# Fil/nd4js

Hardware: AMD Instinct MI355X
Metric: fp64 GFLOP/s: matmul N=4096 & SVD N=2048; % of MFMA/HBM peak (higher is better)
Workload: dtype f64; 1 GPU; matmul 4096x4096x4096 fp64, one matrix pair per GPU (BASELINE configs[1]); parallelism=batch-sharded x1, no collective, inputs=uniform(-1,1) seeds 5/6, HBM-resident

## Files before the change

nd4js_amd/csrc/svd.hip:

```cpp
#include "svd_internal.h"
#include "dpp.h"
#include <cmath>
#include <cfloat>
#include <cstring>

namespace {

constexpr int MAX_SWEEPS = 60;

__device__ __forceinline__ double wave_sum(double v) {
#pragma unroll
  for (int off = 32; off > 0; off >>= 1) v += __shfl_xor(v, off);
  return v;
}

__global__ __launch_bounds__(256) void jac_floor(const double* __restrict__ svr, int N, double tol2, double* __restrict__ floor2) {
  const double* s = svr + (long)blockIdx.x * N;
  double mx = 0.0;
  for (int i = threadIdx.x; i < N; i += 256) mx = fmax(mx, s[i]);
#pragma unroll
  for (int off = 32; off > 0; off >>= 1) mx = fmax(mx, __shfl_xor(mx, off));
  __shared__ double s_mx[4];
  if ((threadIdx.x & 63) == 0) s_mx[threadIdx.x >> 6] = mx;
  __syncthreads();
// ... 209 lines not shown
    __syncthreads();
    const unsigned r = s_rot;
    __syncthreads();
    if (t == 0) s_rot = 0;
    rotations += r;
    converged = r == 0;
    __syncthreads();
  }
  for (int e = t; e < N * N; e += 256) {
    const int r = e / N, c = e % N;
    W[e] = s_w[r * LD + c];
    Ut[e] = s_u[r * LD + c];
  }
  if (t == 0) {
    atomicMax(sweeps_max, (unsigned)sweeps);
    if (!converged) atomicAdd(not_converged, 1u);
    atomicMax(offmax, s_off);
    atomicAdd(rot_total, rotations);
  }
}

int jacobi_square(nd4hip_handle* h, int batch, int N, double* W, double* U, double* sv, double* V,
                  int* sweeps_out, double* offnorm_out) {
  Nd4WsScope scope(h);
  const long sM = (long)N * N;
  void* p = nullptr;
  const bool small = N > 1 && N <= 64;
  const bool blocked = N > 64;
  const int Np = blocked ? ((N + 63) / 64) * 64 : N;
  const bool padded = Np != N;
  const long sMp = (long)Np * Np;
  const size_t nblock = blocked ? nd4_jacobi_block_scratch_doubles(batch, Np) : 0;
  const size_t npad = padded ? (size_t)batch * (2 * sMp + Np) : 0;
  const size_t nd = (size_t)batch * (2 * sM + 2 * N + 1) + nblock + npad;
  const size_t nrank = ((size_t)batch * N + 1) & ~size_t(1);
  ND4_TRY(nd4_ws_alloc(h, nd * sizeof(double) + nrank * sizeof(int) + (size_t)batch * sizeof(JacState) + 96, &p));
  double* Ut = static_cast<double*>(p);
  double* Utp = Ut + (size_t)batch * sM;
  double* svr = Utp + (size_t)batch * sM;
  double* scratch = svr + (size_t)batch * N;
  double* floor2 = scratch + (size_t)batch * N;
  double* bscratch = floor2 + batch;
  double* Wp = bscratch + nblock;
  double* Utpad = Wp + (padded ? (size_t)batch * sMp : 0);
  double* svrp = Utpad + (padded ? (size_t)batch * sMp : 0);
  int* rank = reinterpret_cast<int*>(bscratch + nblock + npad);
  JacState* st = reinterpret_cast<JacState*>(rank + nrank);
  unsigned* active = reinterpret_cast<unsigned*>(st + batch);
  unsigned long long* offmax = reinterpret_cast<unsigned long long*>(active + 2);
  unsigned long long* rot_total = offmax + 1;
  void* pin = nullptr;
  ND4_TRY(nd4_pinned(h, 64 + sizeof(int) * (size_t)batch, &pin));
  unsigned* h_active = static_cast<unsigned*>(pin);
  unsigned long long* h_off = reinterpret_cast<unsigned long long*>(h_active + 2);

  if (!small) ND4_TRY(nd4_set_identity(h, N, N, Ut, N, batch, sM));
  ND4_HIP(hipMemsetAsync(st, 0, sizeof(JacState) * batch + 32, h->stream));
  if (padded) {
    ND4_HIP(hipMemsetAsync(Wp, 0, sizeof(double) * (size_t)batch * sMp, h->stream));
    ND4_TRY(nd4_copy_matrix(h, N, N, W, N, Wp, Np, batch, sM, sMp));
    ND4_TRY(nd4_set_identity(h, Np, Np, Utpad, Np, batch, sMp));
  }
  double* Wb = padded ? Wp : W;
  double* Utb = padded ? Utpad : Ut;

  const double eps = 0x1p-52, tol = N * eps, tol2 = tol * tol;
  if (!small) {
    hipLaunchKernelGGL(jac_norms, dim3((unsigned)((N + 3) / 4), (unsigned)batch), dim3(256), 0, h->stream, W, N, sM, svr);
    hipLaunchKernelGGL(jac_floor, dim3((unsigned)batch), dim3(256), 0, h->stream, svr, N, tol2, floor2);
  }
  int sweeps = 0;
  unsigned long long last_off = 0, rot_seen = 0;
  bool dense_phase = blocked && Np >= 512;
  if (small) {
    ND4_HIP(hipMemsetAsync(active, 0, 16, h->stream));
// ... 189 lines not shown
```

nd4js_amd/csrc/svd_block.hip:

```cpp
#include "svd_internal.h"
#include <cstdlib>

typedef double d4 __attribute__((ext_vector_type(4)));
typedef double d2 __attribute__((ext_vector_type(2)));

namespace {

constexpr int BB = 32;
constexpr int PB = 64;
constexpr int CH = 256;

template <int K> __device__ __forceinline__ int bcast_i(int v) { return __builtin_amdgcn_readlane(v, K); }
template <int K> __device__ __forceinline__ double bcast_d(double v) {
  return __hiloint2double(__builtin_amdgcn_readlane(__double2hiint(v), K), __builtin_amdgcn_readlane(__double2loint(v), K));
}

__device__ __forceinline__ double fast_rcp(double x) {
  double r = __builtin_amdgcn_rcp(x);
  r = fma(fma(-x, r, 1.0), r, r);
  r = fma(fma(-x, r, 1.0), r, r);
  return r;
}
__device__ __forceinline__ double fast_rsqrt(double x) {
  double r = __builtin_amdgcn_rsq(x);
  r = r * fma(-0.5 * x * r, r, 1.5);
  r = r * fma(-0.5 * x * r, r, 1.5);
  return r;
}

__device__ __forceinline__ long pair_row(int x, int I, int J) { return x < BB ? (long)I * BB + x : (long)J * BB + (x - BB); }

__host__ __device__ __forceinline__ void jacb_pair(int n2, int s, int i, int& I, int& J) {
  if (n2 > 0) { nd4_rr_pair(n2, s, i, I, J); return; }
  const int n = -n2, h = n / 2, q = n / 4;
  const int grp = i >= q ? 1 : 0, ii = i - grp * q;
  if (s < h - 1) {
    nd4_rr_pair(h, s, ii, I, J);
    I += grp * h; J += grp * h;
  } else {
    const int c = s - (h - 1), second = c >= q ? 1 : 0, cc = c - second * q;
    I = grp * q + ii;
    J = h + ((grp ^ second) ? q : 0) + (ii + cc) % q;
  }
}
__host__ __device__ __forceinline__ int jacb_abs(int n2) { return n2 < 0 ? -n2 : n2; }

__device__ __forceinline__ void gram_load_group(d2 (&dst)[2][4], const double* const (&rp)[4], int c) {
#pragma unroll
  for (int t = 0; t < 4; t++) {
    dst[0][t] = *reinterpret_cast<const d2*>(rp[t] + c);
    dst[1][t] = *reinterpret_cast<const d2*>(rp[t] + c + 2);
  }
}
__device__ __forceinline__ void gram_mfma_group(d4 (&acc)[4][4], const d2 (&f)[2][4]) {
#pragma unroll
  for (int u = 0; u < 2; u++)
#pragma unroll
    for (int i = 0; i < 4; i++)
#pragma unroll
      for (int j = i; j < 4; j++) {
        acc[i][j] = __builtin_amdgcn_mfma_f64_16x16x4f64(f[u][i].x, f[u][j].x, acc[i][j], 0, 0, 0);
        acc[i][j] = __builtin_amdgcn_mfma_f64_16x16x4f64(f[u][i].y, f[u][j].y, acc[i][j], 0, 0, 0);
      }
}
__device__ __forceinline__ void gram_accumulate(d4 (&acc)[4][4], const double* const (&rp)[4], int col0, int ncols, int N, int fk) {
  for (int c0 = col0; c0 < col0 + ncols && c0 < N; c0 += 16) {
    d2 f[2][4];
    gram_load_group(f, rp, c0 + 4 * fk);
    gram_mfma_group(acc, f);
  }
}
template <int LDG>
__device__ __forceinline__ void gram_reduce_lds(double (*G)[LDG], const d4 (&acc)[4][4], int wave, int fk, int fx) {
#pragma unroll
  for (int w = 0; w < 4; w++) {
    if (wave == w) {
#pragma unroll
      for (int i = 0; i < 4; i++)
#pragma unroll
        for (int j = i; j < 4; j++)
#pragma unroll
          for (int r = 0; r < 4; r++) {
            const int row = i * 16 + fk + 4 * r, col = j * 16 + fx;
            double* d = &G[row][col];
            const double v = (w == 0) ? acc[i][j][r] : *d + acc[i][j][r];
            *d = v;
            if (w == 3 && j > i) G[col][row] = v;
          }
    }
    __syncthreads();
  }
}

template <int NT>
__device__ __forceinline__ void gram2_tiles(d4 (&acc)[3], const double (*st)[PB + 2], const int (&ti)[3], const int (&tj)[3], int fx, int fk) {
#pragma unroll
  for (int ks = 0; ks < 16; ks++) {
    double f[4];
#pragma unroll
    for (int q = 0; q < 4; q++) f[q] = st[q * 16 + fx][ks * 4 + fk];
#pragma unroll
    for (int n = 0; n < NT; n++) acc[n] = __builtin_amdgcn_mfma_f64_16x16x4f64(f[ti[n]], f[tj[n]], acc[n], 0, 0, 0);
  }
}
__global__ __launch_bounds__(256) void jacb_gram2(const double* __restrict__ Wm, int N, long sM, int nblk, int nblk2, int step,
                                                   const JacState* __restrict__ st, double* __restrict__ Gpart, int nchunks, long sG_mat, int pair0) {
  __shared__ double s_x[2][PB][PB + 2];
  const int pairIdx = blockIdx.x + pair0, chunk = blockIdx.y, mat = blockIdx.z;
  if (st[mat].done) return;
  int I, J;
  jacb_pair(nblk2, step, pairIdx, I, J);
  if (J >= nblk) return;
  const double* W = Wm + mat * sM;
  const int t = threadIdx.x, lane = t & 63, wave = __builtin_amdgcn_readfirstlane(t >> 6);
  const int fx = lane & 15, fk = lane >> 4;
  const double* src[8];
#pragma unroll
  for (int k = 0; k < 8; k++) src[k] = W + pair_row((t >> 5) + 8 * k, I, J) * N + chunk * CH + 2 * (t & 31);
  const int nsub = (N - chunk * CH >= CH) ? CH / 64 : (N - chunk * CH) / 64;
  d2 v[8];
  auto load = [&](int sub) {
#pragma unroll
    for (int k = 0; k < 8; k++) v[k] = *reinterpret_cast<const d2*>(src[k] + sub * 64);
  };
  auto stash = [&](int buf) {
#pragma unroll
    for (int k = 0; k < 8; k++) *reinterpret_cast<d2*>(&s_x[buf][(t >> 5) + 8 * k][2 * (t & 31)]) = v[k];
  };
  d4 acc[3] = {d4{0.0, 0.0, 0.0, 0.0}, d4{0.0, 0.0, 0.0, 0.0}, d4{0.0, 0.0, 0.0, 0.0}};
  if (nsub > 0) { load(0); stash(0); }
  __syncthreads();
  for (int sub = 0; sub < nsub; sub++) {
    if (sub + 1 < nsub) load(sub + 1);
    const double (*sx)[PB + 2] = s_x[sub & 1];
    if (wave == 0)      { const int ti[3] = {0, 0, 0}, tj[3] = {0, 1, 2}; gram2_tiles<3>(acc, sx, ti, tj, fx, fk); }
    else if (wave == 1) { const int ti[3] = {0, 1, 1}, tj[3] = {3, 1, 2}; gram2_tiles<3>(acc, sx, ti, tj, fx, fk); }
    else if (wave == 2) { const int ti[3] = {1, 2, 2}, tj[3] = {3, 2, 2}; gram2_tiles<2>(acc, sx, ti, tj, fx, fk); }
    else                { const int ti[3] = {2, 3, 3}, tj[3] = {3, 3, 3}; gram2_tiles<2>(acc, sx, ti, tj, fx, fk); }
    if (sub + 1 < nsub) stash((sub + 1) & 1);
    __syncthreads();
  }
  const int TI[4][3] = {{0, 0, 0}, {0, 1, 1}, {1, 2, 2}, {2, 3, 3}};
  const int TJ[4][3] = {{0, 1, 2}, {3, 1, 2}, {3, 2, 2}, {3, 3, 3}};
  double* G = Gpart + mat * sG_mat + ((long)pairIdx * nchunks + chunk) * (PB * PB);
  const int ntiles = wave < 2 ? 3 : 2;
#pragma unroll
  for (int n = 0; n < 3; n++) {
    if (n < ntiles) {
      const int i = TI[wave][n], j = TJ[wave][n];
#pragma unroll
      for (int r = 0; r < 4; r++) G[(i * 16 + fk + 4 * r) * PB + j * 16 + fx] = acc[n][r];
    }
  }
}

template <bool FUSED, int PW>
__global__ __launch_bounds__(2048 / PW) void jacb_eigen(const double* __restrict__ Gpart, int nchunks, long sG_mat, int nblk, int nblk2, int step,
                                                   JacState* __restrict__ st, const double* __restrict__ floor2, double tol2,
                                                   double* __restrict__ Qt_all, long sQ_mat, int* __restrict__ flags, long sF_mat,
                                                   unsigned long long* __restrict__ offmax, int max_inner, int cross_only) {
  __shared__ double G[PB][PB + 1];
  __shared__ double Q[PB][PB + 1];
  __shared__ unsigned s_rot[32 / PW];
  const int pairIdx = blockIdx.x, mat = blockIdx.y;
  if (st[mat].done) return;
  int I, J;
  jacb_pair(nblk2, step, pairIdx, I, J);
  if (J >= nblk) return;
  const int t = threadIdx.x, lane = t & 63, wave = t >> 6;
  if constexpr (FUSED) {
    static_assert(!FUSED || PW == 8, "the fused Gram phase is written for 4 waves");
    const int N = nchunks, fx = lane & 15, fk = lane >> 4;
    const double* W = Gpart + mat * sG_mat;
    const double* rp[4];
#pragma unroll
    for (int q = 0; q < 4; q++) rp[q] = W + pair_row(q * 16 + fx, I, J) * N;
    d4 acc[4][4];
#pragma unroll
    for (int i = 0; i < 4; i++)
#pragma unroll
      for (int j = 0; j < 4; j++) acc[i][j] = d4{0.0, 0.0, 0.0, 0.0};
    const int per = ((N + 63) / 64) * 16;
    gram_accumulate(acc, rp, wave * per, per, N, fk);
    gram_reduce_lds<PB + 1>(G, acc, wave, fk, fx);
    for (int e = t; e < PB * PB; e += 2048 / PW) Q[e / PB][e % PB] = (e / PB == e % PB) ? 1.0 : 0.0;
  } else {
    const double* Gp = Gpart + mat * sG_mat + (long)pairIdx * nchunks * (PB * PB);
    for (int e = t; e < PB * PB; e += 2048 / PW) {
      const int r = e / PB, c = e % PB;
      Q[r][c] = (r == c) ? 1.0 : 0.0;
      if ((r >> 4) > (c >> 4)) continue;
      double s = 0.0;
      for (int ch = 0; ch < nchunks; ch++) s += Gp[(long)ch * (PB * PB) + e];
      G[r][c] = s;
      if ((r >> 4) != (c >> 4)) G[c][r] = s;
    }
  }
  __syncthreads();
  const double fl = floor2[mat];
  unsigned total = 0;
  double relmax = 0.0;
  {
    int need = 0;
    for (int e = t; e < PB * PB; e += 2048 / PW) {
      const int i = e / PB, j = e % PB;
      if (i < j) { const double a = G[i][i], b = G[j][j], g = G[i][j]; need |= (a > fl) && (b > fl) && (g * g > tol2 * a * b); }
    }
    need = __syncthreads_or(need);
    if (!need) { if (t == 0) flags[mat * sF_mat + pairIdx] = 0; return; }
  }
  const int nrounds = cross_only ? BB : PB - 1;
  for (int inner = 0; inner < max_inner; inner++) {
    unsigned rot = 0;
    for (int r = 0; r < nrounds; r++) {
      int p, q;
      if (cross_only) { p = wave * PW + (lane & (PW - 1)); q = BB + ((p + r) & (BB - 1)); }
      else nd4_rr_pair(PB, r, wave * PW + (lane & (PW - 1)), p, q);
      const double a = G[p][p], b = G[q][q], g = G[p][q];
      const bool go = (a > fl) && (b > fl) && (g * g > tol2 * a * b);
      double c = 1.0, s = 0.0;
      if (go) {
        const double d = b - a, hh = 2.0 * g, rr = d * d + hh * hh;
        const double root = rr * fast_rsqrt(rr);
        const double tn = (((d < 0.0) != (g < 0.0)) ? -fabs(hh) : fabs(hh)) * fast_rcp(fabs(d) + root);
        const double cc = fast_rsqrt(1.0 + tn * tn);
        s = cc * tn;
// ... 43 lines not shown
  double* Qt = Qt_all + mat * sQ_mat + (long)pairIdx * (PB * PB);
  if (total) for (int e = t; e < PB * PB; e += 2048 / PW) Qt[e] = Q[e / PB][e % PB];
#pragma unroll
  for (int off = 32; off > 0; off >>= 1) relmax = fmax(relmax, __shfl_xor(relmax, off));
  if (lane == 0 && relmax > 0.0) atomicMax(offmax, (unsigned long long)__double_as_longlong(relmax));
  if (t == 0) {
    flags[mat * sF_mat + pairIdx] = total ? 1 : 0;
    if (total) atomicAdd(&st[mat].rotations, total);
  }
}

template <int CG>
__device__ __forceinline__ void eigen_p_body(double* __restrict__ stage_raw, const int pairIdx, const int mat,
                                             const double* __restrict__ Gpart, int nchunks, long sG_mat, int nblk, int nblk2, int step,
                                             JacState* __restrict__ st, const double* __restrict__ floor2, double tol2,
                                             double* __restrict__ Qt_all, long sQ_mat, int* __restrict__ flags, long sF_mat,
                                             unsigned long long* __restrict__ offmax, int precheck) {
  constexpr int T = 576, TB = 512, NB = 2, NQ = 4;
  constexpr int LD = BB + 1;
  __shared__ double sC[2][BB][LD];
  __shared__ double sB[2][BB][LD];
  __shared__ double sA1[2][BB];
  __shared__ double sAng[2][2][BB];
  double (*stage)[PB + 1] = reinterpret_cast<double (*)[PB + 1]>(stage_raw);
  __shared__ double sRd[PB];
  __shared__ unsigned sTotal;
  double (*QJ)[PB + 1] = stage;
  if (st[mat].done) return;
  int I, J;
  jacb_pair(nblk2, step, pairIdx, I, J);
  if (J >= nblk) return;
  const int t = threadIdx.x, lane = t & 63, wave = t >> 6;
  if (t < TB) {
    constexpr int KL = (PB * PB / 2) / TB;
    const d2* Gp = reinterpret_cast<const d2*>(Gpart + mat * sG_mat + (long)pairIdx * nchunks * (PB * PB));
    d2 acc[KL];
#pragma unroll
    for (int k = 0; k < KL; k++) acc[k] = d2{0.0, 0.0};
    for (int ch0 = 0; ch0 < nchunks; ch0 += CG) {
      d2 v[CG][KL];
#pragma unroll
      for (int c = 0; c < CG; c++)
#pragma unroll
        for (int k = 0; k < KL; k++) {
          const int e = 2 * (t + TB * k);
          v[c][k] = (ch0 + c < nchunks && ((e / PB) >> 4) <= ((e % PB) >> 4)) ? Gp[(long)(ch0 + c) * (PB * PB / 2) + t + TB * k] : d2{0.0, 0.0};
        }
#pragma unroll
      for (int c = 0; c < CG; c++)
#pragma unroll
        for (int k = 0; k < KL; k++) acc[k] += v[c][k];
    }
#pragma unroll
    for (int k = 0; k < KL; k++) {
      const int e = 2 * (t + TB * k), r = e / PB, c = e % PB;
      if ((r >> 4) <= (c >> 4)) {
        stage[r][c] = acc[k].x;
        stage[r][c + 1] = acc[k].y;
        if ((r >> 4) != (c >> 4)) { stage[c][r] = acc[k].x; stage[c + 1][r] = acc[k].y; }
      }
    }
  }
  __syncthreads();
  const double fl = floor2[mat];
  if (precheck) {
    if (t < PB) { const double dd = stage[t][t]; sRd[t] = dd > fl ? __builtin_amdgcn_rcp(dd) : 0.0; }
    __syncthreads();
    double rel = 0.0;
    for (int e = t; e < PB * PB; e += T) {
      const int x = e / PB, y = e % PB;
      const double g = stage[x][y];
      if (x < y) rel = fmax(rel, g * g * sRd[x] * sRd[y]);
    }
#pragma unroll
    for (int off = 32; off > 0; off >>= 1) rel = fmax(rel, __shfl_xor(rel, off));
    if (lane == 0 && rel > 0.0) atomicMax(offmax, (unsigned long long)__double_as_longlong(rel));
    const int need = __syncthreads_or(rel > tol2 * (1.0 - 0x1p-20));
    if (!need) { if (t == 0) flags[mat * sF_mat + pairIdx] = 0; return; }
  }
  const int i = lane & 31, h = lane >> 5;
  const bool pivot = wave == 8;
  const int jb = NB * (2 * wave + h);
  const int cb = NQ * (2 * wave + h);
  double Areg[NB] = {0.0, 0.0}, Qp[NQ] = {0.0, 0.0, 0.0, 0.0};
  double pa = 0.0, pb = 0.0, pg = 0.0;
  if (pivot) {
    pa = stage[i][i]; pb = stage[BB + i][BB + i]; pg = stage[i][BB + i];
  } else {
#pragma unroll
    for (int m = 0; m < NB; m++) Areg[m] = stage[i][jb + m];
#pragma unroll
    for (int m = 0; m < NQ; m++) Qp[m] = (cb + m == i) ? 1.0 : 0.0;
// ... 81 lines not shown
  if (t == 8 * 64) sTotal = rot;
  __syncthreads();
  const unsigned total = sTotal;
  if (total) {
    double* Qt = Qt_all + mat * sQ_mat + (long)pairIdx * (PB * PB);
    if (!pivot) {
#pragma unroll
      for (int m = 0; m < NQ; m++) Qt[i * PB + cb + m] = Qp[m];
    }
    for (int e = t; e < BB * PB; e += T) Qt[BB * PB + e] = QJ[e / PB][e % PB];
  }
  if (t == 0) {
    flags[mat * sF_mat + pairIdx] = total ? 1 : 0;
    if (total) atomicAdd(&st[mat].rotations, total);
  }
}

constexpr int SQ_LD = PB + 4;
constexpr int STAGE_DOUBLES = PB * SQ_LD;
template <int T, int STRIPS = 4>
__device__ __forceinline__ void apply_body(double* __restrict__ sq_raw, const int pairIdx, int chunk, const int mat,
                                           double* __restrict__ Wm, double* __restrict__ Utm, int N, long sM, int nblk, int nblk2, int step,
                                           const JacState* __restrict__ st, const double* __restrict__ Qt_all, long sQ_mat,
                                           const int* __restrict__ flags, long sF_mat, int nchunks) {
  double (*sQ)[SQ_LD] = reinterpret_cast<double (*)[SQ_LD]>(sq_raw);
  if (st[mat].done || !flags[mat * sF_mat + pairIdx]) return;
  int I, J;
  jacb_pair(nblk2, step, pairIdx, I, J);
  if (J >= nblk) return;
  double* X = (chunk < nchunks ? Wm : Utm) + mat * sM;
  if (chunk >= nchunks) chunk -= nchunks;
  const int t = threadIdx.x, lane = t & 63, wave = t >> 6;
  const int fx = lane & 15, fk = lane >> 4;
  const double* Qt = Qt_all + mat * sQ_mat + (long)pairIdx * (PB * PB);
  for (int e = t; e < PB * PB; e += T) sQ[e / PB][e % PB] = Qt[e];
  __syncthreads();
  if (T > 256 && t >= 256) return;
  long rowoff[16];
#pragma unroll
  for (int ks = 0; ks < 16; ks++) rowoff[ks] = pair_row(ks * 4 + fk, I, J) * N;
  const int colw = chunk * (64 * STRIPS) + wave * (16 * STRIPS);
  for (int strip = 0; strip < STRIPS; strip++) {
    const int cbase = colw + strip * 16;
    if (cbase >= N) break;
    const int c = cbase + fx;
    double b[16];
#pragma unroll
    for (int ks = 0; ks < 16; ks++) b[ks] = X[rowoff[ks] + c];
#pragma unroll
    for (int it = 0; it < 4; it++) {
      d4 acc = d4{0.0, 0.0, 0.0, 0.0};
#pragma unroll
      for (int ks = 0; ks < 16; ks++)
        acc = __builtin_amdgcn_mfma_f64_16x16x4f64(sQ[it * 16 + fx][ks * 4 + fk], b[ks], acc, 0, 0, 0);
#pragma unroll
      for (int r = 0; r < 4; r++) X[pair_row(it * 16 + fk + 4 * r, I, J) * N + c] = acc[r];
    }
  }
}

__global__ __launch_bounds__(576) void jacb_eigen_p(const double* __restrict__ Gpart, int nchunks, long sG_mat, int nblk, int nblk2, int step,
                                                     JacState* __restrict__ st, const double* __restrict__ floor2, double tol2,
                                                     double* __restrict__ Qt_all, long sQ_mat, int* __restrict__ flags, long sF_mat,
                                                     unsigned long long* __restrict__ offmax, int precheck, int pair0) {
  __shared__ double stage_raw[STAGE_DOUBLES];
  eigen_p_body<4>(stage_raw, blockIdx.x + pair0, blockIdx.y, Gpart, nchunks, sG_mat, nblk, nblk2, step, st, floor2, tol2, Qt_all, sQ_mat, flags, sF_mat,
               offmax, precheck);
}

__global__ __launch_bounds__(256) void jacb_apply(double* __restrict__ Wm, double* __restrict__ Utm, int N, long sM, int nblk, int nblk2, int step,
                                                   const JacState* __restrict__ st, const double* __restrict__ Qt_all, long sQ_mat,
                                                   const int* __restrict__ flags, long sF_mat, int nchunks, int chunk0, int pair0) {
  __shared__ double sq_raw[STAGE_DOUBLES];
  apply_body<256>(sq_raw, blockIdx.x + pair0, blockIdx.y + chunk0, blockIdx.z, Wm, Utm, N, sM, nblk, nblk2, step, st, Qt_all, sQ_mat, flags, sF_mat, nchunks);
}

template <int STRIPS>
__global__ __launch_bounds__(256) void jacb_apply_w(double* __restrict__ Wm, int N, long sM, int nblk, int nblk2, int step,
                                                     const JacState* __restrict__ st, const double* __restrict__ Qt_all, long sQ_mat,
                                                     const int* __restrict__ flags, long sF_mat, int pair0) {
  __shared__ double sq_raw[STAGE_DOUBLES];
  apply_body<256, STRIPS>(sq_raw, blockIdx.x + pair0, blockIdx.y, blockIdx.z, Wm, nullptr, N, sM, nblk, nblk2, step, st, Qt_all, sQ_mat, flags, sF_mat,
                          (int)gridDim.y);
}

__global__ __launch_bounds__(576) void jacb_eigen_pu(const double* __restrict__ Gpart, int nchunks, long sG_mat, int nblk, int nblk2, int step,
                                                      JacState* __restrict__ st, const double* __restrict__ floor2, double tol2,
                                                      double* __restrict__ Qt_all, long sQ_mat, int* __restrict__ flags, long sF_mat,
                                                      unsigned long long* __restrict__ offmax, int precheck, int npairs,
                                                      double* __restrict__ Utm, int N, long sM, const double* __restrict__ Qt_prev,
                                                      const int* __restrict__ flags_prev, int pair0) {
  __shared__ double stage_raw[STAGE_DOUBLES];
  if ((int)blockIdx.x < npairs) {
    eigen_p_body<8>(stage_raw, blockIdx.x + pair0, blockIdx.y, Gpart, nchunks, sG_mat, nblk, nblk2, step, st, floor2, tol2, Qt_all, sQ_mat, flags, sF_mat,
                 offmax, precheck);
  } else {
    const int idx = (int)blockIdx.x - npairs;
    apply_body<576>(stage_raw, idx % npairs + pair0, nchunks + idx / npairs, blockIdx.y, nullptr, Utm, N, sM, nblk, nblk2, step - 1, st, Qt_prev, sQ_mat,
                    flags_prev, sF_mat, nchunks);
  }
}

}

size_t nd4_jacobi_block_scratch_doubles(int batch, int N) {
  const int nblk = N / BB, nblk2 = (nblk + 1) & ~1, npairs = nblk2 / 2, nchunks = (N + CH - 1) / CH;
  const size_t per = (size_t)npairs * nchunks * PB * PB + 2 * ((size_t)npairs * PB * PB + (size_t)((npairs + 1) / 2 + 1));
  return per * batch;
}

namespace {

struct JacbSweep {
  nd4hip_handle* h;
  int batch, N; double* W; double* Ut; JacState* st; const double* floor2; double tol2; unsigned long long* offmax;
  int precheck;
  int nblk, npairs, nchunks;
  long sM, sG, sQ, sF;
  double* Gpart; double* Qt2[2]; int* flags2[2];
  int wstrips;
};

void jacb_launch_apply_w(const JacbSweep& s, hipStream_t stream, int n2, int step, int np, int batch, double* Qt, int* flags, int p0) {
  if (s.wstrips == 1)
    hipLaunchKernelGGL(jacb_apply_w<1>, dim3((unsigned)np, (unsigned)(s.N / 64), (unsigned)batch), dim3(256), 0, stream,
                       s.W, s.N, s.sM, s.nblk, n2, step, s.st, Qt, s.sQ, flags, s.sF, p0);
  else
    hipLaunchKernelGGL(jacb_apply_w<2>, dim3((unsigned)np, (unsigned)((s.N + 127) / 128), (unsigned)batch), dim3(256), 0, stream,
                       s.W, s.N, s.sM, s.nblk, n2, step, s.st, Qt, s.sQ, flags, s.sF, p0);
}

int jacb_sweep_two_chains(const JacbSweep& s) {
  nd4hip_handle* h = s.h;
  const int N = s.N, nblk = s.nblk, npairs = s.npairs, nchunks = s.nchunks;
  const int n2 = -nblk, hq = nblk / 2, q = nblk / 4, nsteps = nblk - 1;
  hipStream_t chain[2] = {h->stream, h->aux_stream};
  hipLaunchKernelGGL(jacb_gram2, dim3((unsigned)npairs, (unsigned)nchunks, 1u), dim3(256), 0, chain[0], s.W, N, s.sM, nblk, n2, 0, s.st, s.Gpart, nchunks, s.sG, 0);
  hipLaunchKernelGGL((jacb_eigen<false, 2>), dim3((unsigned)npairs, 1u), dim3(1024), 0, chain[0],
                     s.Gpart, nchunks, s.sG, nblk, n2, 0, s.st, s.floor2, s.tol2, s.Qt2[0], s.sQ, s.flags2[0], s.sF, s.offmax, 1, 0);
  hipLaunchKernelGGL(jacb_apply, dim3((unsigned)npairs, (unsigned)(2 * nchunks), 1u), dim3(256), 0, chain[0],
                     s.W, s.Ut, N, s.sM, nblk, n2, 0, s.st, s.Qt2[0], s.sQ, s.flags2[0], s.sF, nchunks, 0, 0);
  ND4_HIP(hipEventRecord(h->ev_aux_a, chain[0]));
  ND4_HIP(hipStreamWaitEvent(chain[1], h->ev_aux_a, 0));
  bool prev_full = true;
  for (int step = 1; step < nsteps; step++) {
    const bool phase_end = step == hq - 2 || step == hq - 2 + q || step == nsteps - 1;
    double* Qt = s.Qt2[step & 1];
    int* flags = s.flags2[step & 1];
    for (int c = 0; c < 2; c++) {
      const int p0 = c * q;
      hipLaunchKernelGGL(jacb_gram2, dim3((unsigned)q, (unsigned)nchunks, 1u), dim3(256), 0, chain[c], s.W, N, s.sM, nblk, n2, step, s.st, s.Gpart, nchunks, s.sG, p0);
      if (prev_full)
        hipLaunchKernelGGL(jacb_eigen_p, dim3((unsigned)q, 1u), dim3(576), 0, chain[c],
                           s.Gpart, nchunks, s.sG, nblk, n2, step, s.st, s.floor2, s.tol2, Qt, s.sQ, flags, s.sF, s.offmax, s.precheck, p0);
      else
        hipLaunchKernelGGL(jacb_eigen_pu, dim3((unsigned)(q + q * nchunks), 1u), dim3(576), 0, chain[c],
                           s.Gpart, nchunks, s.sG, nblk, n2, step, s.st, s.floor2, s.tol2, Qt, s.sQ, flags, s.sF, s.offmax, s.precheck, q,
                           s.Ut, N, s.sM, s.Qt2[(step - 1) & 1], s.flags2[(step - 1) & 1], p0);
      if (phase_end)
        hipLaunchKernelGGL(jacb_apply, dim3((unsigned)q, (unsigned)(2 * nchunks), 1u), dim3(256), 0, chain[c],
                           s.W, s.Ut, N, s.sM, nblk, n2, step, s.st, Qt, s.sQ, flags, s.sF, nchunks, 0, p0);
      else
        jacb_launch_apply_w(s, chain[c], n2, step, q, 1, Qt, flags, p0);
    }
    prev_full = phase_end;
    if (phase_end) {
      ND4_HIP(hipEventRecord(h->ev_aux_a, chain[0]));
      ND4_HIP(hipEventRecord(h->ev_aux_b, chain[1]));
      ND4_HIP(hipStreamWaitEvent(chain[1], h->ev_aux_a, 0));
      ND4_HIP(hipStreamWaitEvent(chain[0], h->ev_aux_b, 0));
    }
  }
  ND4_HIP(hipGetLastError());
  return 0;
}

int jacb_sweep_one_chain(const JacbSweep& s, const bool defer) {
  nd4hip_handle* h = s.h;
  const int N = s.N, batch = s.batch, nblk = s.nblk, nblk2 = (nblk + 1) & ~1, npairs = s.npairs, nchunks = s.nchunks;
  const bool fused = N <= 1024 && batch * npairs >= 128 && batch * npairs <= 768;
  for (int step = 0; step < nblk2 - 1; step++) {
    const bool cross_only = step > 0;
    double* Qt = s.Qt2[defer ? (step & 1) : 0];
    int* flags = s.flags2[defer ? (step & 1) : 0];
    const bool last = step == nblk2 - 2;
    if (fused) {
      hipLaunchKernelGGL((jacb_eigen<true, 8>), dim3((unsigned)npairs, (unsigned)batch), dim3(256), 0, h->stream,
                         s.W, N, s.sM, nblk, nblk2, step, s.st, s.floor2, s.tol2, Qt, s.sQ, flags, s.sF, s.offmax, 1, cross_only ? 1 : 0);
    } else {
      hipLaunchKernelGGL(jacb_gram2, dim3((unsigned)npairs, (unsigned)nchunks, (unsigned)batch), dim3(256), 0, h->stream,
                         s.W, N, s.sM, nblk, nblk2, step, s.st, s.Gpart, nchunks, s.sG, 0);
      if (cross_only && defer) {
        hipLaunchKernelGGL(jacb_eigen_pu, dim3((unsigned)(npairs + npairs * nchunks), (unsigned)batch), dim3(576), 0, h->stream,
                           s.Gpart, nchunks, s.sG, nblk, nblk2, step, s.st, s.floor2, s.tol2, Qt, s.sQ, flags, s.sF, s.offmax, s.precheck, npairs,
                           s.Ut, N, s.sM, s.Qt2[(step - 1) & 1], s.flags2[(step - 1) & 1], 0);
      } else if (cross_only) {
        hipLaunchKernelGGL(jacb_eigen_p, dim3((unsigned)npairs, (unsigned)batch), dim3(576), 0, h->stream,
                           s.Gpart, nchunks, s.sG, nblk, nblk2, step, s.st, s.floor2, s.tol2, Qt, s.sQ, flags, s.sF, s.offmax, s.precheck, 0);
      } else if ((long)batch * npairs <= 256) {
        hipLaunchKernelGGL((jacb_eigen<false, 2>), dim3((unsigned)npairs, (unsigned)batch), dim3(1024), 0, h->stream,
                           s.Gpart, nchunks, s.sG, nblk, nblk2, step, s.st, s.floor2, s.tol2, Qt, s.sQ, flags, s.sF, s.offmax, 1, 0);
      } else {
        hipLaunchKernelGGL((jacb_eigen<false, 8>), dim3((unsigned)npairs, (unsigned)batch), dim3(256), 0, h->stream,
                           s.Gpart, nchunks, s.sG, nblk, nblk2, step, s.st, s.floor2, s.tol2, Qt, s.sQ, flags, s.sF, s.offmax, 1, 0);
      }
    }
    if (defer && !last)
      jacb_launch_apply_w(s, h->stream, nblk2, step, npairs, batch, Qt, flags, 0);
    else
      hipLaunchKernelGGL(jacb_apply, dim3((unsigned)npairs, (unsigned)(2 * nchunks), (unsigned)batch), dim3(256), 0, h->stream,
                         s.W, s.Ut, N, s.sM, nblk, nblk2, step, s.st, Qt, s.sQ, flags, s.sF, nchunks, 0, 0);
  }
  ND4_HIP(hipGetLastError());
  return 0;
}

}

int nd4_jacobi_block_sweep(nd4hip_handle* h, int batch, int N, double* W, double* Ut, JacState* st,
                           const double* floor2, double tol2, unsigned long long* offmax, double* scratch, bool dense_phase) {
  JacbSweep s;
  s.h = h; s.batch = batch; s.N = N; s.W = W; s.Ut = Ut; s.st = st; s.floor2 = floor2; s.tol2 = tol2; s.offmax = offmax;
  s.precheck = dense_phase ? 0 : 1;
  s.nblk = N / BB; s.npairs = ((s.nblk + 1) & ~1) / 2; s.nchunks = (N + CH - 1) / CH;
  s.sM = (long)N * N;
  s.sG = (long)s.npairs * s.nchunks * PB * PB; s.sQ = (long)s.npairs * PB * PB;
  s.sF = ((s.npairs + 1) / 2 + 1) * 2;
  s.Gpart = scratch;
  s.Qt2[0] = s.Gpart + (size_t)batch * s.sG;
  s.flags2[0] = reinterpret_cast<int*>(s.Qt2[0] + (size_t)batch * s.sQ);
  s.Qt2[1] = s.Qt2[0] + (size_t)batch * s.sQ + (size_t)batch * (s.sF / 2);
  s.flags2[1] = reinterpret_cast<int*>(s.Qt2[1] + (size_t)batch * s.sQ);
  s.wstrips = N <= 2048 ? 1 : 2;
  const bool defer = (long)batch * s.npairs <= 64 && N >= 512;
  const char* two_e = getenv("ND4HIP_JAC_TWO_CHAINS");
  const int two_min_n = two_e ? atoi(two_e) : 4096;
  if (two_min_n > 0 && defer && batch == 1 && s.nblk % 4 == 0 && N >= two_min_n) return jacb_sweep_two_chains(s);
  return jacb_sweep_one_chain(s, defer);
}
```

Before: 75970 GFLOP/s.

## Spread Gram tile MFMAs over 8 waves and vectorize Qt staging loads

The Gram kernel now launches 512 threads (8 waves) instead of 256. Each wave computes one or two 16x16 tiles of the 10 upper-triangle tiles instead of two or three, and each thread loads half as many rows per sub-chunk. The Qt load into shared memory in the apply path now uses 16-byte d2 vector loads, and shared buffers plus scratch offsets are padded and aligned to keep those vector accesses 16-byte aligned. This targets the latency-bound Gram step of the blocked Jacobi SVD, at the cost of uneven load across waves and more register and occupancy pressure per block.

```diff
diff --git a/nd4js_amd/csrc/svd.hip b/nd4js_amd/csrc/svd.hip
--- a/nd4js_amd/csrc/svd.hip
+++ b/nd4js_amd/csrc/svd.hip
@@ -265,7 +265,7 @@
   const long sMp = (long)Np * Np;
   const size_t nblock = blocked ? nd4_jacobi_block_scratch_doubles(batch, Np) : 0;
   const size_t npad = padded ? (size_t)batch * (2 * sMp + Np) : 0;
-  const size_t nd = (size_t)batch * (2 * sM + 2 * N + 1) + nblock + npad;
+  const size_t nd = (size_t)batch * (2 * sM + 2 * N + 1) + (batch & 1) + nblock + npad;
   const size_t nrank = ((size_t)batch * N + 1) & ~size_t(1);
   ND4_TRY(nd4_ws_alloc(h, nd * sizeof(double) + nrank * sizeof(int) + (size_t)batch * sizeof(JacState) + 96, &p));
   double* Ut = static_cast<double*>(p);
@@ -273,7 +273,7 @@
   double* svr = Utp + (size_t)batch * sM;
   double* scratch = svr + (size_t)batch * N;
   double* floor2 = scratch + (size_t)batch * N;
-  double* bscratch = floor2 + batch;
+  double* bscratch = floor2 + batch + (batch & 1);
   double* Wp = bscratch + nblock;
   double* Utpad = Wp + (padded ? (size_t)batch * sMp : 0);
   double* svrp = Utpad + (padded ? (size_t)batch * sMp : 0);
diff --git a/nd4js_amd/csrc/svd_block.hip b/nd4js_amd/csrc/svd_block.hip
--- a/nd4js_amd/csrc/svd_block.hip
+++ b/nd4js_amd/csrc/svd_block.hip
@@ -92,20 +92,19 @@
   }
 }
 
+constexpr int GRAM_T = 512;
 template <int NT>
-__device__ __forceinline__ void gram2_tiles(d4 (&acc)[3], const double (*st)[PB + 2], const int (&ti)[3], const int (&tj)[3], int fx, int fk) {
+__device__ __forceinline__ void gram2_tiles(d4 (&acc)[2], const double (*st)[PB + 2], int ti, int tj0, int tj1, int fx, int fk) {
 #pragma unroll
   for (int ks = 0; ks < 16; ks++) {
-    double f[4];
-#pragma unroll
-    for (int q = 0; q < 4; q++) f[q] = st[q * 16 + fx][ks * 4 + fk];
-#pragma unroll
-    for (int n = 0; n < NT; n++) acc[n] = __builtin_amdgcn_mfma_f64_16x16x4f64(f[ti[n]], f[tj[n]], acc[n], 0, 0, 0);
-  }
-}
-__global__ __launch_bounds__(256) void jacb_gram2(const double* __restrict__ Wm, int N, long sM, int nblk, int nblk2, int step,
-                                                   const JacState* __restrict__ st, double* __restrict__ Gpart, int nchunks, long sG_mat, int pair0) {
-  __shared__ double s_x[2][PB][PB + 2];
+    const double fa = st[ti * 16 + fx][ks * 4 + fk], fb = st[tj0 * 16 + fx][ks * 4 + fk];
+    acc[0] = __builtin_amdgcn_mfma_f64_16x16x4f64(fa, fb, acc[0], 0, 0, 0);
+    if constexpr (NT > 1) acc[1] = __builtin_amdgcn_mfma_f64_16x16x4f64(fa, st[tj1 * 16 + fx][ks * 4 + fk], acc[1], 0, 0, 0);
+  }
+}
+__global__ __launch_bounds__(GRAM_T) void jacb_gram2(const double* __restrict__ Wm, int N, long sM, int nblk, int nblk2, int step,
+                                                      const JacState* __restrict__ st, double* __restrict__ Gpart, int nchunks, long sG_mat, int pair0) {
+  __shared__ __attribute__((aligned(16))) double s_x[2][PB][PB + 2];
   const int pairIdx = blockIdx.x + pair0, chunk = blockIdx.y, mat = blockIdx.z;
   if (st[mat].done) return;
   int I, J;
@@ -114,43 +113,41 @@
   const double* W = Wm + mat * sM;
   const int t = threadIdx.x, lane = t & 63, wave = __builtin_amdgcn_readfirstlane(t >> 6);
   const int fx = lane & 15, fk = lane >> 4;
-  const double* src[8];
-#pragma unroll
-  for (int k = 0; k < 8; k++) src[k] = W + pair_row((t >> 5) + 8 * k, I, J) * N + chunk * CH + 2 * (t & 31);
+  const double* src[4];
+#pragma unroll
+  for (int k = 0; k < 4; k++) src[k] = W + pair_row((t >> 5) + 16 * k, I, J) * N + chunk * CH + 2 * (t & 31);
   const int nsub = (N - chunk * CH >= CH) ? CH / 64 : (N - chunk * CH) / 64;
-  d2 v[8];
+  d2 v[4];
   auto load = [&](int sub) {
 #pragma unroll
-    for (int k = 0; k < 8; k++) v[k] = *reinterpret_cast<const d2*>(src[k] + sub * 64);
+    for (int k = 0; k < 4; k++) v[k] = *reinterpret_cast<const d2*>(src[k] + sub * 64);
   };
   auto stash = [&](int buf) {
 #pragma unroll
-    for (int k = 0; k < 8; k++) *reinterpret_cast<d2*>(&s_x[buf][(t >> 5) + 8 * k][2 * (t & 31)]) = v[k];
+    for (int k = 0; k < 4; k++) *reinterpret_cast<d2*>(&s_x[buf][(t >> 5) + 16 * k][2 * (t & 31)]) = v[k];
   };
-  d4 acc[3] = {d4{0.0, 0.0, 0.0, 0.0}, d4{0.0, 0.0, 0.0, 0.0}, d4{0.0, 0.0, 0.0, 0.0}};
+  constexpr int TI[8]  =    {0, 0, 0, 1, 1, 1, 2, 3};
+  constexpr int TJ0[8] =    {0, 2, 3, 1, 2, 3, 2, 3};
+  constexpr int TJ1[8] =    {1, 0, 0, 0, 0, 0, 3, 0};
+  const int ti = TI[wave], tj0 = TJ0[wave], tj1 = TJ1[wave];
+  const bool two = wave == 0 || wave == 6;
+  d4 acc[2] = {d4{0.0, 0.0, 0.0, 0.0}, d4{0.0, 0.0, 0.0, 0.0}};
   if (nsub > 0) { load(0); stash(0); }
   __syncthreads();
   for (int sub = 0; sub < nsub; sub++) {
     if (sub + 1 < nsub) load(sub + 1);
     const double (*sx)[PB + 2] = s_x[sub & 1];
-    if (wave == 0)      { const int ti[3] = {0, 0, 0}, tj[3] = {0, 1, 2}; gram2_tiles<3>(acc, sx, ti, tj, fx, fk); }
-    else if (wave == 1) { const int ti[3] = {0, 1, 1}, tj[3] = {3, 1, 2}; gram2_tiles<3>(acc, sx, ti, tj, fx, fk); }
-    else if (wave == 2) { const int ti[3] = {1, 2, 2}, tj[3] = {3, 2, 2}; gram2_tiles<2>(acc, sx, ti, tj, fx, fk); }
-    else                { const int ti[3] = {2, 3, 3}, tj[3] = {3, 3, 3}; gram2_tiles<2>(acc, sx, ti, tj, fx, fk); }
+    if (two) gram2_tiles<2>(acc, sx, ti, tj0, tj1, fx, fk);
+    else     gram2_tiles<1>(acc, sx, ti, tj0, tj1, fx, fk);
     if (sub + 1 < nsub) stash((sub + 1) & 1);
     __syncthreads();
   }
-  const int TI[4][3] = {{0, 0, 0}, {0, 1, 1}, {1, 2, 2}, {2, 3, 3}};
-  const int TJ[4][3] = {{0, 1, 2}, {3, 1, 2}, {3, 2, 2}, {3, 3, 3}};
   double* G = Gpart + mat * sG_mat + ((long)pairIdx * nchunks + chunk) * (PB * PB);
-  const int ntiles = wave < 2 ? 3 : 2;
-#pragma unroll
-  for (int n = 0; n < 3; n++) {
-    if (n < ntiles) {
-      const int i = TI[wave][n], j = TJ[wave][n];
-#pragma unroll
-      for (int r = 0; r < 4; r++) G[(i * 16 + fk + 4 * r) * PB + j * 16 + fx] = acc[n][r];
-    }
+#pragma unroll
+  for (int r = 0; r < 4; r++) G[(ti * 16 + fk + 4 * r) * PB + tj0 * 16 + fx] = acc[0][r];
+  if (two) {
+#pragma unroll
+    for (int r = 0; r < 4; r++) G[(ti * 16 + fk + 4 * r) * PB + tj1 * 16 + fx] = acc[1][r];
   }
 }
 
@@ -475,7 +472,8 @@
   const int t = threadIdx.x, lane = t & 63, wave = t >> 6;
   const int fx = lane & 15, fk = lane >> 4;
   const double* Qt = Qt_all + mat * sQ_mat + (long)pairIdx * (PB * PB);
-  for (int e = t; e < PB * PB; e += T) sQ[e / PB][e % PB] = Qt[e];
+  for (int e = t; e < PB * PB / 2; e += T)
+    *reinterpret_cast<d2*>(&sQ[e / (PB / 2)][2 * (e % (PB / 2))]) = reinterpret_cast<const d2*>(Qt)[e];
   __syncthreads();
   if (T > 256 && t >= 256) return;
   long rowoff[16];
@@ -505,7 +503,7 @@
                                                      JacState* __restrict__ st, const double* __restrict__ floor2, double tol2,
                                                      double* __restrict__ Qt_all, long sQ_mat, int* __restrict__ flags, long sF_mat,
                                                      unsigned long long* __restrict__ offmax, int precheck, int pair0) {
-  __shared__ double stage_raw[STAGE_DOUBLES];
+  __shared__ __attribute__((aligned(16))) double stage_raw[STAGE_DOUBLES];
   eigen_p_body<4>(stage_raw, blockIdx.x + pair0, blockIdx.y, Gpart, nchunks, sG_mat, nblk, nblk2, step, st, floor2, tol2, Qt_all, sQ_mat, flags, sF_mat,
                offmax, precheck);
 }
@@ -513,7 +511,7 @@
 __global__ __launch_bounds__(256) void jacb_apply(double* __restrict__ Wm, double* __restrict__ Utm, int N, long sM, int nblk, int nblk2, int step,
                                                    const JacState* __restrict__ st, const double* __restrict__ Qt_all, long sQ_mat,
                                                    const int* __restrict__ flags, long sF_mat, int nchunks, int chunk0, int pair0) {
-  __shared__ double sq_raw[STAGE_DOUBLES];
+  __shared__ __attribute__((aligned(16))) double sq_raw[STAGE_DOUBLES];
   apply_body<256>(sq_raw, blockIdx.x + pair0, blockIdx.y + chunk0, blockIdx.z, Wm, Utm, N, sM, nblk, nblk2, step, st, Qt_all, sQ_mat, flags, sF_mat, nchunks);
 }
 
@@ -521,7 +519,7 @@
 __global__ __launch_bounds__(256) void jacb_apply_w(double* __restrict__ Wm, int N, long sM, int nblk, int nblk2, int step,
                                                      const JacState* __restrict__ st, const double* __restrict__ Qt_all, long sQ_mat,
                                                      const int* __restrict__ flags, long sF_mat, int pair0) {
-  __shared__ double sq_raw[STAGE_DOUBLES];
+  __shared__ __attribute__((aligned(16))) double sq_raw[STAGE_DOUBLES];
   apply_body<256, STRIPS>(sq_raw, blockIdx.x + pair0, blockIdx.y, blockIdx.z, Wm, nullptr, N, sM, nblk, nblk2, step, st, Qt_all, sQ_mat, flags, sF_mat,
                           (int)gridDim.y);
 }
@@ -532,7 +530,7 @@
                                                       unsigned long long* __restrict__ offmax, int precheck, int npairs,
                                                       double* __restrict__ Utm, int N, long sM, const double* __restrict__ Qt_prev,
                                                       const int* __restrict__ flags_prev, int pair0) {
-  __shared__ double stage_raw[STAGE_DOUBLES];
+  __shared__ __attribute__((aligned(16))) double stage_raw[STAGE_DOUBLES];
   if ((int)blockIdx.x < npairs) {
     eigen_p_body<8>(stage_raw, blockIdx.x + pair0, blockIdx.y, Gpart, nchunks, sG_mat, nblk, nblk2, step, st, floor2, tol2, Qt_all, sQ_mat, flags, sF_mat,
                  offmax, precheck);
@@ -547,7 +545,7 @@
 
 size_t nd4_jacobi_block_scratch_doubles(int batch, int N) {
   const int nblk = N / BB, nblk2 = (nblk + 1) & ~1, npairs = nblk2 / 2, nchunks = (N + CH - 1) / CH;
-  const size_t per = (size_t)npairs * nchunks * PB * PB + 2 * ((size_t)npairs * PB * PB + (size_t)((npairs + 1) / 2 + 1));
+  const size_t per = (size_t)npairs * nchunks * PB * PB + 2 * ((size_t)npairs * PB * PB + (size_t)(((npairs + 1) / 2 + 2) & ~1));
   return per * batch;
 }
 
@@ -577,7 +575,7 @@
   const int N = s.N, nblk = s.nblk, npairs = s.npairs, nchunks = s.nchunks;
   const int n2 = -nblk, hq = nblk / 2, q = nblk / 4, nsteps = nblk - 1;
   hipStream_t chain[2] = {h->stream, h->aux_stream};
-  hipLaunchKernelGGL(jacb_gram2, dim3((unsigned)npairs, (unsigned)nchunks, 1u), dim3(256), 0, chain[0], s.W, N, s.sM, nblk, n2, 0, s.st, s.Gpart, nchunks, s.sG, 0);
+  hipLaunchKernelGGL(jacb_gram2, dim3((unsigned)npairs, (unsigned)nchunks, 1u), dim3(GRAM_T), 0, chain[0], s.W, N, s.sM, nblk, n2, 0, s.st, s.Gpart, nchunks, s.sG, 0);
   hipLaunchKernelGGL((jacb_eigen<false, 2>), dim3((unsigned)npairs, 1u), dim3(1024), 0, chain[0],
                      s.Gpart, nchunks, s.sG, nblk, n2, 0, s.st, s.floor2, s.tol2, s.Qt2[0], s.sQ, s.flags2[0], s.sF, s.offmax, 1, 0);
   hipLaunchKernelGGL(jacb_apply, dim3((unsigned)npairs, (unsigned)(2 * nchunks), 1u), dim3(256), 0, chain[0],
@@ -591,7 +589,7 @@
     int* flags = s.flags2[step & 1];
     for (int c = 0; c < 2; c++) {
       const int p0 = c * q;
-      hipLaunchKernelGGL(jacb_gram2, dim3((unsigned)q, (unsigned)nchunks, 1u), dim3(256), 0, chain[c], s.W, N, s.sM, nblk, n2, step, s.st, s.Gpart, nchunks, s.sG, p0);
+      hipLaunchKernelGGL(jacb_gram2, dim3((unsigned)q, (unsigned)nchunks, 1u), dim3(GRAM_T), 0, chain[c], s.W, N, s.sM, nblk, n2, step, s.st, s.Gpart, nchunks, s.sG, p0);
       if (prev_full)
         hipLaunchKernelGGL(jacb_eigen_p, dim3((unsigned)q, 1u), dim3(576), 0, chain[c],
                            s.Gpart, nchunks, s.sG, nblk, n2, step, s.st, s.floor2, s.tol2, Qt, s.sQ, flags, s.sF, s.offmax, s.precheck, p0);
@@ -630,7 +628,7 @@
       hipLaunchKernelGGL((jacb_eigen<true, 8>), dim3((unsigned)npairs, (unsigned)batch), dim3(256), 0, h->stream,
                          s.W, N, s.sM, nblk, nblk2, step, s.st, s.floor2, s.tol2, Qt, s.sQ, flags, s.sF, s.offmax, 1, cross_only ? 1 : 0);
     } else {
-      hipLaunchKernelGGL(jacb_gram2, dim3((unsigned)npairs, (unsigned)nchunks, (unsigned)batch), dim3(256), 0, h->stream,
+      hipLaunchKernelGGL(jacb_gram2, dim3((unsigned)npairs, (unsigned)nchunks, (unsigned)batch), dim3(GRAM_T), 0, h->stream,
                          s.W, N, s.sM, nblk, nblk2, step, s.st, s.Gpart, nchunks, s.sG, 0);
       if (cross_only && defer) {
         hipLaunchKernelGGL(jacb_eigen_pu, dim3((unsigned)(npairs + npairs * nchunks), (unsigned)batch), dim3(576), 0, h->stream,
@@ -667,7 +665,7 @@
   s.nblk = N / BB; s.npairs = ((s.nblk + 1) & ~1) / 2; s.nchunks = (N + CH - 1) / CH;
   s.sM = (long)N * N;
   s.sG = (long)s.npairs * s.nchunks * PB * PB; s.sQ = (long)s.npairs * PB * PB;
-  s.sF = ((s.npairs + 1) / 2 + 1) * 2;
+  s.sF = (((s.npairs + 1) / 2 + 2) & ~1) * 2;
   s.Gpart = scratch;
   s.Qt2[0] = s.Gpart + (size_t)batch * s.sG;
   s.flags2[0] = reinterpret_cast<int*>(s.Qt2[0] + (size_t)batch * s.sQ);
```

New measurement: 76000 GFLOP/s (median of 4 runs). About the same (+0.0%).

## Pack Gram partials into compact upper-tile layout with vectorized stores and loads

Applied to the files above, without the earlier changes.

Gram partial tiles are now stored as 10 packed 16x16 upper-triangle tiles per chunk in lane order instead of a full 64x64 strided matrix. The writer can then emit contiguous 16-byte stores and the reducers read only live data, which removes the wasted lower-triangle traffic and the scattered writes. The Qt load into LDS is vectorized as well, and the scratch and shared buffers are 16/128-byte aligned so these wide accesses are legal. The row/col decode in the reducers gets more complex, and a mismatch between writer and reader layouts would silently corrupt results.

```diff
diff --git a/nd4js_amd/csrc/svd_block.hip b/nd4js_amd/csrc/svd_block.hip
--- a/nd4js_amd/csrc/svd_block.hip
+++ b/nd4js_amd/csrc/svd_block.hip
@@ -1,4 +1,5 @@
 #include "svd_internal.h"
+#include <cstdint>
 #include <cstdlib>
 
 typedef double d4 __attribute__((ext_vector_type(4)));
@@ -29,6 +30,19 @@
 }
 
 __device__ __forceinline__ long pair_row(int x, int I, int J) { return x < BB ? (long)I * BB + x : (long)J * BB + (x - BB); }
+
+constexpr int GP_TILES = 10, GP_DOUBLES = GP_TILES * 256;
+__device__ __forceinline__ void gp_tile_ij(int tile, int& i, int& j) {
+  i = (int)(0x3221110000ULL >> (4 * tile)) & 3;
+  j = (int)(0x3323213210ULL >> (4 * tile)) & 3;
+}
+__device__ __forceinline__ void gp_row_col(int e, int& row, int& col) {
+  int i, j;
+  gp_tile_ij(e >> 8, i, j);
+  const int l = (e >> 2) & 63;
+  row = i * 16 + (l >> 4) + 4 * (e & 3);
+  col = j * 16 + (l & 15);
+}
 
 __host__ __device__ __forceinline__ void jacb_pair(int n2, int s, int i, int& I, int& J) {
   if (n2 > 0) { nd4_rr_pair(n2, s, i, I, J); return; }
@@ -140,16 +154,14 @@
     if (sub + 1 < nsub) stash((sub + 1) & 1);
     __syncthreads();
   }
-  const int TI[4][3] = {{0, 0, 0}, {0, 1, 1}, {1, 2, 2}, {2, 3, 3}};
-  const int TJ[4][3] = {{0, 1, 2}, {3, 1, 2}, {3, 2, 2}, {3, 3, 3}};
-  double* G = Gpart + mat * sG_mat + ((long)pairIdx * nchunks + chunk) * (PB * PB);
-  const int ntiles = wave < 2 ? 3 : 2;
+  double* G = Gpart + mat * sG_mat + ((long)pairIdx * nchunks + chunk) * GP_DOUBLES;
+  const int ntiles = wave < 2 ? 3 : 2, tile0 = wave < 2 ? 3 * wave : 2 * wave + 2;
 #pragma unroll
   for (int n = 0; n < 3; n++) {
     if (n < ntiles) {
-      const int i = TI[wave][n], j = TJ[wave][n];
-#pragma unroll
-      for (int r = 0; r < 4; r++) G[(i * 16 + fk + 4 * r) * PB + j * 16 + fx] = acc[n][r];
+      d2* g = reinterpret_cast<d2*>(G + (tile0 + n) * 256 + 4 * lane);
+      g[0] = d2{acc[n][0], acc[n][1]};
+      g[1] = d2{acc[n][2], acc[n][3]};
     }
   }
 }
@@ -185,13 +197,13 @@
     gram_reduce_lds<PB + 1>(G, acc, wave, fk, fx);
     for (int e = t; e < PB * PB; e += 2048 / PW) Q[e / PB][e % PB] = (e / PB == e % PB) ? 1.0 : 0.0;
   } else {
-    const double* Gp = Gpart + mat * sG_mat + (long)pairIdx * nchunks * (PB * PB);
-    for (int e = t; e < PB * PB; e += 2048 / PW) {
-      const int r = e / PB, c = e % PB;
-      Q[r][c] = (r == c) ? 1.0 : 0.0;
-      if ((r >> 4) > (c >> 4)) continue;
+    const double* Gp = Gpart + mat * sG_mat + (long)pairIdx * nchunks * GP_DOUBLES;
+    for (int e = t; e < PB * PB; e += 2048 / PW) Q[e / PB][e % PB] = (e / PB == e % PB) ? 1.0 : 0.0;
+    for (int e = t; e < GP_DOUBLES; e += 2048 / PW) {
+      int r, c;
+      gp_row_col(e, r, c);
       double s = 0.0;
-      for (int ch = 0; ch < nchunks; ch++) s += Gp[(long)ch * (PB * PB) + e];
+      for (int ch = 0; ch < nchunks; ch++) s += Gp[(long)ch * GP_DOUBLES + e];
       G[r][c] = s;
       if ((r >> 4) != (c >> 4)) G[c][r] = s;
     }
@@ -301,8 +313,8 @@
   if (J >= nblk) return;
   const int t = threadIdx.x, lane = t & 63, wave = t >> 6;
   if (t < TB) {
-    constexpr int KL = (PB * PB / 2) / TB;
-    const d2* Gp = reinterpret_cast<const d2*>(Gpart + mat * sG_mat + (long)pairIdx * nchunks * (PB * PB));
+    constexpr int KL = (GP_DOUBLES / 2 + TB - 1) / TB;
+    const d2* Gp = reinterpret_cast<const d2*>(Gpart + mat * sG_mat + (long)pairIdx * nchunks * GP_DOUBLES);
     d2 acc[KL];
 #pragma unroll
     for (int k = 0; k < KL; k++) acc[k] = d2{0.0, 0.0};
@@ -311,10 +323,8 @@
 #pragma unroll
       for (int c = 0; c < CG; c++)
 #pragma unroll
-        for (int k = 0; k < KL; k++) {
-          const int e = 2 * (t + TB * k);
-          v[c][k] = (ch0 + c < nchunks && ((e / PB) >> 4) <= ((e % PB) >> 4)) ? Gp[(long)(ch0 + c) * (PB * PB / 2) + t + TB * k] : d2{0.0, 0.0};
-        }
+        for (int k = 0; k < KL; k++)
+          v[c][k] = (ch0 + c < nchunks && t + TB * k < GP_DOUBLES / 2) ? Gp[(long)(ch0 + c) * (GP_DOUBLES / 2) + t + TB * k] : d2{0.0, 0.0};
 #pragma unroll
       for (int c = 0; c < CG; c++)
 #pragma unroll
@@ -322,11 +332,12 @@
     }
 #pragma unroll
     for (int k = 0; k < KL; k++) {
-      const int e = 2 * (t + TB * k), r = e / PB, c = e % PB;
-      if ((r >> 4) <= (c >> 4)) {
+      if (t + TB * k < GP_DOUBLES / 2) {
+        int r, c;
+        gp_row_col(2 * (t + TB * k), r, c);
         stage[r][c] = acc[k].x;
-        stage[r][c + 1] = acc[k].y;
-        if ((r >> 4) != (c >> 4)) { stage[c][r] = acc[k].x; stage[c + 1][r] = acc[k].y; }
+        stage[r + 4][c] = acc[k].y;
+        if ((r >> 4) != (c >> 4)) { stage[c][r] = acc[k].x; stage[c][r + 4] = acc[k].y; }
       }
     }
   }
@@ -474,8 +485,16 @@
   if (chunk >= nchunks) chunk -= nchunks;
   const int t = threadIdx.x, lane = t & 63, wave = t >> 6;
   const int fx = lane & 15, fk = lane >> 4;
-  const double* Qt = Qt_all + mat * sQ_mat + (long)pairIdx * (PB * PB);
-  for (int e = t; e < PB * PB; e += T) sQ[e / PB][e % PB] = Qt[e];
+  const d2* Qt = reinterpret_cast<const d2*>(Qt_all + mat * sQ_mat + (long)pairIdx * (PB * PB));
+  constexpr int QL = (PB * PB / 2 + T - 1) / T;
+  d2 q[QL];
+#pragma unroll
+  for (int k = 0; k < QL; k++) if (T * (k + 1) <= PB * PB / 2 || t + T * k < PB * PB / 2) q[k] = Qt[t + T * k];
+#pragma unroll
+  for (int k = 0; k < QL; k++) {
+    const int e = t + T * k;
+    if (T * (k + 1) <= PB * PB / 2 || e < PB * PB / 2) *reinterpret_cast<d2*>(&sQ[e / (PB / 2)][2 * (e % (PB / 2))]) = q[k];
+  }
   __syncthreads();
   if (T > 256 && t >= 256) return;
   long rowoff[16];
@@ -505,7 +524,7 @@
                                                      JacState* __restrict__ st, const double* __restrict__ floor2, double tol2,
                                                      double* __restrict__ Qt_all, long sQ_mat, int* __restrict__ flags, long sF_mat,
                                                      unsigned long long* __restrict__ offmax, int precheck, int pair0) {
-  __shared__ double stage_raw[STAGE_DOUBLES];
+  __shared__ alignas(16) double stage_raw[STAGE_DOUBLES];
   eigen_p_body<4>(stage_raw, blockIdx.x + pair0, blockIdx.y, Gpart, nchunks, sG_mat, nblk, nblk2, step, st, floor2, tol2, Qt_all, sQ_mat, flags, sF_mat,
                offmax, precheck);
 }
@@ -513,7 +532,7 @@
 __global__ __launch_bounds__(256) void jacb_apply(double* __restrict__ Wm, double* __restrict__ Utm, int N, long sM, int nblk, int nblk2, int step,
                                                    const JacState* __restrict__ st, const double* __restrict__ Qt_all, long sQ_mat,
                                                    const int* __restrict__ flags, long sF_mat, int nchunks, int chunk0, int pair0) {
-  __shared__ double sq_raw[STAGE_DOUBLES];
+  __shared__ alignas(16) double sq_raw[STAGE_DOUBLES];
   apply_body<256>(sq_raw, blockIdx.x + pair0, blockIdx.y + chunk0, blockIdx.z, Wm, Utm, N, sM, nblk, nblk2, step, st, Qt_all, sQ_mat, flags, sF_mat, nchunks);
 }
 
@@ -521,7 +540,7 @@
 __global__ __launch_bounds__(256) void jacb_apply_w(double* __restrict__ Wm, int N, long sM, int nblk, int nblk2, int step,
                                                      const JacState* __restrict__ st, const double* __restrict__ Qt_all, long sQ_mat,
                                                      const int* __restrict__ flags, long sF_mat, int pair0) {
-  __shared__ double sq_raw[STAGE_DOUBLES];
+  __shared__ alignas(16) double sq_raw[STAGE_DOUBLES];
   apply_body<256, STRIPS>(sq_raw, blockIdx.x + pair0, blockIdx.y, blockIdx.z, Wm, nullptr, N, sM, nblk, nblk2, step, st, Qt_all, sQ_mat, flags, sF_mat,
                           (int)gridDim.y);
 }
@@ -532,7 +551,7 @@
                                                       unsigned long long* __restrict__ offmax, int precheck, int npairs,
                                                       double* __restrict__ Utm, int N, long sM, const double* __restrict__ Qt_prev,
                                                       const int* __restrict__ flags_prev, int pair0) {
-  __shared__ double stage_raw[STAGE_DOUBLES];
+  __shared__ alignas(16) double stage_raw[STAGE_DOUBLES];
   if ((int)blockIdx.x < npairs) {
     eigen_p_body<8>(stage_raw, blockIdx.x + pair0, blockIdx.y, Gpart, nchunks, sG_mat, nblk, nblk2, step, st, floor2, tol2, Qt_all, sQ_mat, flags, sF_mat,
                  offmax, precheck);
@@ -545,10 +564,12 @@
 
 }
 
+constexpr size_t SCRATCH_ALIGN = 128;
+static int jacb_flag_ints(int npairs) { return (npairs + 3) & ~3; }
 size_t nd4_jacobi_block_scratch_doubles(int batch, int N) {
   const int nblk = N / BB, nblk2 = (nblk + 1) & ~1, npairs = nblk2 / 2, nchunks = (N + CH - 1) / CH;
-  const size_t per = (size_t)npairs * nchunks * PB * PB + 2 * ((size_t)npairs * PB * PB + (size_t)((npairs + 1) / 2 + 1));
-  return per * batch;
+  const size_t per = (size_t)npairs * nchunks * GP_DOUBLES + 2 * ((size_t)npairs * PB * PB + (size_t)(jacb_flag_ints(npairs) / 2));
+  return per * batch + SCRATCH_ALIGN / sizeof(double);
 }
 
 namespace {
@@ -666,9 +687,9 @@
   s.precheck = dense_phase ? 0 : 1;
   s.nblk = N / BB; s.npairs = ((s.nblk + 1) & ~1) / 2; s.nchunks = (N + CH - 1) / CH;
   s.sM = (long)N * N;
-  s.sG = (long)s.npairs * s.nchunks * PB * PB; s.sQ = (long)s.npairs * PB * PB;
-  s.sF = ((s.npairs + 1) / 2 + 1) * 2;
-  s.Gpart = scratch;
+  s.sG = (long)s.npairs * s.nchunks * GP_DOUBLES; s.sQ = (long)s.npairs * PB * PB;
+  s.sF = jacb_flag_ints(s.npairs);
+  s.Gpart = reinterpret_cast<double*>((reinterpret_cast<uintptr_t>(scratch) + (SCRATCH_ALIGN - 1)) & ~(uintptr_t)(SCRATCH_ALIGN - 1));
   s.Qt2[0] = s.Gpart + (size_t)batch * s.sG;
   s.flags2[0] = reinterpret_cast<int*>(s.Qt2[0] + (size_t)batch * s.sQ);
   s.Qt2[1] = s.Qt2[0] + (size_t)batch * s.sQ + (size_t)batch * (s.sF / 2);
```

Result: no change. 75620 GFLOP/s before, 75490 GFLOP/s after (-0.2%).
